# qwertyhgb/Prostate-Cancer-Multimodal-Segmentation

Measured on AMD Instinct MI355X. Metric: train volumes/sec (5ch 128x128x64), higher is better.
Workload: dtype bf16; 1 GPU; UNet3D 5->1, 2 x 5x128x128x64 per GPU, BCEDiceLoss, Adam(1e-4, wd 1e-5); global_batch=2, parallelism=dp1

## Files before the change

include/pcms_hip.h:

```cpp
#ifndef PCMS_HIP_H
#define PCMS_HIP_H
#include <hip/hip_runtime.h>

#ifdef __cplusplus
extern "C" {
#endif

#define PCMS_CONV_ACCUMULATE 1
#define PCMS_CONV_RELU 2
#define PCMS_GRAD_STORE 1
#define PCMS_STEM_DENSE 16

int pcms_pack_input(int dtype, const float* in, void* out, int N, int Cin, long V, int Cp, hipStream_t s);

int pcms_conv3_chunk(int dtype);
int pcms_conv3_pack_elems(int dtype, int J, int Kdim);
int pcms_conv3_mblocks(int N, int D, int H, int W);
int pcms_conv3_fwd_rows(int dtype, int N, int D, int H, int W, int c0, int c1, int Cout);
int pcms_conv3_big_min_boxes(int v);
int pcms_conv3_big_max_wgs(int v);
int pcms_conv3_small_box_mtw2(int v);
int pcms_conv3_fwd_box_vol(int v);
int pcms_conv3_pack(int dtype, const float* w, void* out, int Cout, int Cin, int flip, hipStream_t s);
int pcms_conv3_pack2(int dtype, const float* w, void* fwd, void* dgrad, int Cout, int Cin, hipStream_t s);
// ... 75 lines not shown
int pcms_maxpool_fwd(int dtype, const void* a, void* p, int N, int D, int H, int W, int C, hipStream_t s);
int pcms_maxpool_bwd(int dtype, const void* a, const void* dp, void* da, int N, int D, int H, int W,
                     int C, hipStream_t s);
int pcms_bn_relu_pool(int dtype, const void* y, void* a, void* p, const float* scale, const float* shift,
                      int N, int D, int H, int W, int C, hipStream_t s);
int pcms_maxpool_bwd_bn_rows(int dtype, int N, int D, int H, int W, int C);
int pcms_maxpool_bwd_bn(int dtype, const void* y, const float* scale, const float* shift, const float* mean,
                        const float* invstd, const void* dp, void* da, float* part, int N, int D, int H, int W,
                        int C, hipStream_t s);
int pcms_maxpool_bwd_bn_sums(int dtype, const void* y, const float* scale, const float* shift, const float* mean,
                             const float* invstd, const void* dp, const void* da, float* part, int N, int D, int H,
                             int W, int C, hipStream_t s);
int pcms_maxpool_bn_apply(int dtype, const void* y, const float* scale, const float* shift, const float* mean,
                          const float* invstd, const float* coef, const void* dp, const void* da, void* dy, int N,
                          int D, int H, int W, int C, hipStream_t s);

int pcms_convt_fwd_stream(int v);
int pcms_convt_pack_elems(int dtype, int Cin, int Cout);
int pcms_convt_pack(int dtype, const float* w, void* out, int Cin, int Cout, int dgrad, hipStream_t s);
int pcms_convt_fwd(int dtype, const void* x, const void* wpack, const float* bias, void* out,
                   int N, int Din, int Hin, int Win, int Cin, int Cout, int Do, int Ho, int Wo, hipStream_t s);
int pcms_convt_fwd_ws_floats(int N, int Din, int Hin, int Win, int Cin, int Cout);
int pcms_convt_fwd_ws(int dtype, const void* x, const void* wpack, const float* bias, void* out, float* ws,
                      int N, int Din, int Hin, int Win, int Cin, int Cout, int Do, int Ho, int Wo, hipStream_t s);
int pcms_convt_dgrad(int dtype, const void* dout, const void* wpack_d, void* dx,
                     int N, int Din, int Hin, int Win, int Cin, int Cout, int Do, int Ho, int Wo, hipStream_t s);
int pcms_convt_dgrad_ws_floats(int N, int Din, int Hin, int Win, int Cin, int Cout);
int pcms_convt_dgrad_ws(int dtype, const void* dout, const void* wpack_d, void* dx, float* ws,
                        int N, int Din, int Hin, int Win, int Cin, int Cout, int Do, int Ho, int Wo, hipStream_t s);
int pcms_convt_wgrad_ws_floats(int N, int Din, int Hin, int Win, int Cin, int Cout, int target_wgs);
// ... 89 lines not shown
```

prostate-cancer-multimodal-segmentation_amd/_lib.py:

```python
from __future__ import annotations

import ctypes
import os

import torch

LIB_PATH = os.environ.get("PCMS_LIB") or os.path.join(os.path.dirname(os.path.abspath(__file__)), "libpcms_hip.so")

F32, BF16, F32X3 = 0, 1, 2

SIGNATURES = {
    "pcms_pack_input": "ippiilis",
    "pcms_conv3_chunk": "i",
    "pcms_conv3_pack_elems": "iii",
    "pcms_conv3_mblocks": "iiii",
    "pcms_conv3_fwd_rows": "iiiiiiii",
    "pcms_conv3_big_min_boxes": "i",
    "pcms_conv3_big_max_wgs": "i",
    "pcms_conv3_fwd_box_vol": "i",
    "pcms_conv3_small_box_mtw2": "i",
    "pcms_conv3_pack": "ippiiis",
    "pcms_conv3_pack2": "ipppiis",
    "pcms_conv3_splits": "iii",
    "pcms_conv3_fwd": "ipipippppippiiiiiiis",
# ... 32 lines not shown
    "pcms_split_epilogue": "ipipppipilis",
    "pcms_bn_ws_doubles": "i",
    "pcms_bn_finalize": "piidpppppffppppps",
    "pcms_bn_eval_coeffs": "ppppfipps",
    "pcms_bn_fold": "ppppppfilpps",
    "pcms_bn_relu": "ippppils",
    "pcms_bn_bwd_rows": "iil",
    "pcms_bn_relu_bwd": "i" + "p" * 12 + "ilps",
    "pcms_maxpool_fwd": "ippiiiiis",
    "pcms_maxpool_bwd": "ipppiiiiis",
    "pcms_bn_relu_pool": "ipppppiiiiis",
    "pcms_maxpool_bwd_bn_rows": "iiiiii",
    "pcms_maxpool_bwd_bn": "ippppppppiiiiis",
    "pcms_maxpool_bwd_bn_sums": "ippppppppiiiiis",
    "pcms_maxpool_bn_apply": "ipppppppppiiiiis",
    "pcms_bn_relu_bwd_finish": "i" + "p" * 8 + "ippppilps",
    "pcms_convt_pack": "ippiiis",
    "pcms_convt_pack_elems": "iii",
    "pcms_convt_fwd_stream": "i",
    "pcms_convt_fwd": "ippppiiiiiiiiis",
    "pcms_convt_fwd_ws_floats": "iiiiii",
    "pcms_convt_fwd_ws": "ipppppiiiiiiiiis",
    "pcms_convt_dgrad": "ipppiiiiiiiiis",
    "pcms_convt_dgrad_ws_floats": "iiiiii",
    "pcms_convt_dgrad_ws": "ippppiiiiiiiiis",
    "pcms_convt_wgrad_ws_floats": "iiiiiii",
    "pcms_convt_wgrad_taps": "i",
    "pcms_convt_reduce_fused": "i",
    "pcms_bn_bwd_rows_cap": "i",
    "pcms_convt_wgrad": "ippppiiiiiiiiiis",
# ... 111 lines not shown
```

prostate-cancer-multimodal-segmentation_amd/csrc/ops.hip:

```cpp
#include "common.h"
#include "pcms_hip.h"
#include <algorithm>

namespace {

constexpr int TPB = 256;

template <typename T>
__global__ void pack_input_kernel(const float* in, T* out, int N, int Cin, long V, int Cp) {
  const long total = (long)N * V;
  for (long i = blockIdx.x * (long)blockDim.x + threadIdx.x; i < total; i += (long)gridDim.x * blockDim.x) {
    const long n = i / V, v = i % V;
    for (int c = 0; c < Cp; ++c) {
      const float x = c < Cin ? in[(n * Cin + c) * V + v] : 0.f;
      Elem<T>::st(out + i * Cp + c, x);
    }
  }
}

template <typename T>
__global__ void __launch_bounds__(256) pack_input4_kernel(const float* in, T* out, int N, int Cin, long V) {
  const long quads = (long)N * V / 4;
  for (long i = blockIdx.x * (long)blockDim.x + threadIdx.x; i < quads; i += (long)gridDim.x * blockDim.x) {
    const long n = (4 * i) / V, v = (4 * i) % V;
// ... 371 lines not shown
      for (int j = 0; j < VEC; ++j)
        if (v[j] > m[j] || (v[j] != v[j] && m[j] == m[j])) { m[j] = v[j]; arg[j] = k; }
    }
    float g[VEC];
    load16<T>(dp + i * VEC, g);
    for (int k = 0; k < 8; ++k) {
      float o[VEC];
      load16<T>(da + vin[k] * C + cv * VEC, o);
#pragma unroll
      for (int j = 0; j < VEC; ++j) o[j] += (arg[j] == k) ? g[j] : 0.f;
      store16<T>(da + vin[k] * C + cv * VEC, o);
    }
  }
}

template <typename T, bool NT>
__global__ void __launch_bounds__(TPB) bn_relu_pool_kernel(const T* y, T* a, T* p, const float* scale,
                                                           const float* shift, int N, int D, int H, int W,
                                                           int C) {
  constexpr int VEC = Elem<T>::kVec;
  const int Dc = (D + 1) / 2, Hc = (H + 1) / 2, Wc = (W + 1) / 2, CV = C / VEC;
  const int Do = D / 2, Ho = H / 2, Wo = W / 2;
  const long total = (long)N * Dc * Hc * Wc * CV;
  const long stride = (long)gridDim.x * blockDim.x;
  long i = blockIdx.x * (long)blockDim.x + threadIdx.x;
  const int cv = (int)(i % CV);
  float sc[VEC], sh[VEC];
#pragma unroll
  for (int j = 0; j < VEC; ++j) { sc[j] = scale[cv * VEC + j]; sh[j] = shift[cv * VEC + j]; }
  for (; i < total; i += stride) {
    uint32_t r = (uint32_t)(i / CV);
    const int wc = r % Wc; r /= Wc;
    const int hc = r % Hc; r /= Hc;
    const int dc = r % Dc; const long n = r / Dc;
    float m[VEC];
#pragma unroll
    for (int j = 0; j < VEC; ++j) m[j] = -INFINITY;
    float v[8][VEC];
    long vin[8];
    bool in[8];
#pragma unroll
    for (int k = 0; k < 8; ++k) {
      const int d = 2 * dc + (k >> 2), h = 2 * hc + ((k >> 1) & 1), w = 2 * wc + (k & 1);
      in[k] = d < D && h < H && w < W;
      vin[k] = ((n * D + d) * H + h) * W + w;
#ifndef BRP_NTLOAD
#define BRP_NTLOAD 1
#endif
      if (in[k]) ld16<NT && BRP_NTLOAD>(y + vin[k] * C + cv * VEC, v[k]);
    }
#pragma unroll
    for (int k = 0; k < 8; ++k) {
      if (!in[k]) continue;
#pragma unroll
      for (int j = 0; j < VEC; ++j) v[k][j] = round_st<T>(bn_relu1(v[k][j], sc[j], sh[j]));
      st16<NT>(a + vin[k] * C + cv * VEC, v[k]);
#pragma unroll
      for (int j = 0; j < VEC; ++j)
        if (v[k][j] > m[j] || v[k][j] != v[k][j]) m[j] = v[k][j];
    }
    if (dc < Do && hc < Ho && wc < Wo) store16<T>(p + (((n * Do + dc) * Ho + hc) * Wo + wc) * C + cv * VEC, m);
  }
}

template <typename T, bool STORE = true>
__global__ void __launch_bounds__(TPB, 3) maxpool_bwd_bn_kernel(const T* y, const float* scale, const float* shift,
                                                             const float* mean, const float* invstd, const T* dp,
                                                             T* da, float* part, int N, int D, int H, int W,
                                                             int C) {
  constexpr int VEC = Elem<T>::kVec;
  __shared__ float red[TPB][VEC][2];
  const int Dc = (D + 1) / 2, Hc = (H + 1) / 2, Wc = (W + 1) / 2, CV = C / VEC;
  const int Do = D / 2, Ho = H / 2, Wo = W / 2;
  const long total = (long)N * Dc * Hc * Wc * CV;
  const long stride = (long)gridDim.x * blockDim.x;
  long i = blockIdx.x * (long)blockDim.x + threadIdx.x;
  const int cv = (int)(i % CV);
  float sc[VEC], sh[VEC], mu[VEC], is[VEC], sg[VEC], sgx[VEC];
#pragma unroll
  for (int j = 0; j < VEC; ++j) {
    const int c = cv * VEC + j;
    sc[j] = scale[c]; sh[j] = shift[c]; mu[j] = mean[c]; is[j] = invstd[c];
    sg[j] = 0.f; sgx[j] = 0.f;
  }
// ... 14 lines not shown
    const bool whole = dc < Do && hc < Ho && wc < Wo;
    u32x4_t yr[8], dr[8], gr = {0u, 0u, 0u, 0u};
    const long v0 = ((n * D + 2 * dc) * H + 2 * hc) * W + 2 * wc;
    const bool ind = 2 * dc + 1 < D, inh = 2 * hc + 1 < H, inw = 2 * wc + 1 < W;
    auto vk = [&](int k) { return v0 + (long)(k >> 2) * H * W + ((k >> 1) & 1) * W + (k & 1); };
    auto ink = [&](int k) { return (!(k & 4) || ind) && (!(k & 2) || inh) && (!(k & 1) || inw); };
#pragma unroll
    for (int k = 0; k < 8; ++k) {
      yr[k] = (u32x4_t){0u, 0u, 0u, 0u};
      dr[k] = yr[k];
      if (ink(k)) {
        yr[k] = *reinterpret_cast<const u32x4_t*>(y + vk(k) * C + cv * VEC);
        dr[k] = *reinterpret_cast<const u32x4_t*>(da + vk(k) * C + cv * VEC);
      }
    }
    if (whole) gr = *reinterpret_cast<const u32x4_t*>(dp + (((n * Do + dc) * Ho + hc) * Wo + wc) * C + cv * VEC);
    float g[VEC], m[VEC];
    int arg[VEC];
    unpack(gr, g);
#pragma unroll
    for (int j = 0; j < VEC; ++j) { m[j] = -INFINITY; arg[j] = 0; }
    auto round2 = [](f32x2_t v) -> f32x2_t {
      if constexpr (sizeof(T) == 2) {
        const uint32_t u = pack_bf16x2(v[0], v[1]);
        return (f32x2_t){__uint_as_float(u << 16), __uint_as_float(u & 0xffff0000u)};
      } else {
        return v;
      }
    };
    auto z2of = [&](const float (&yv)[VEC], int q) {
      return __builtin_elementwise_fma((f32x2_t){yv[2 * q], yv[2 * q + 1]}, (f32x2_t){sc[2 * q], sc[2 * q + 1]},
                                       (f32x2_t){sh[2 * q], sh[2 * q + 1]});
    };
    if (whole) {
#pragma unroll
      for (int k = 0; k < 8; ++k) {
        float yv[VEC];
        unpack(yr[k], yv);
#pragma unroll
        for (int j = 0; j < VEC; ++j) {
          const float av = round_st<T>(bn_relu1(yv[j], sc[j], sh[j]));
          if (av > m[j] || (av != av && m[j] == m[j])) { m[j] = av; arg[j] = k; }
        }
      }
    }
#pragma unroll
    for (int k = 0; k < 8; ++k) {
      if (!ink(k)) continue;
      float yv[VEC], o[VEC];
// ... 111 lines not shown
    for (int k = 0; k < 8; ++k) {
      if (!ink(k)) continue;
      float yv[VEC], o[VEC], out[VEC];
      u32x4_t yk = yr[k];
      asm volatile("" : "+v"(yk));
      unpack(yk, yv);
      unpack(dr[k], o);
      if (whole) {
#pragma unroll
        for (int j = 0; j < VEC; ++j) o[j] = round_st<T>(o[j] + ((arg[j] == k) ? g[j] : 0.f));
      }
#pragma unroll
      for (int j = 0; j < VEC; ++j) out[j] = bn_bwd_dy(o[j], yv[j], sc[j], sh[j], mu[j], is[j], k1[j], k2[j], k3[j]);
      st16<NT>(dy + vk(k) * C + cv * VEC, out);
    }
  }
}

template <typename T>
__global__ void __launch_bounds__(TPB) box_channel_sum_kernel(const T* x, float* part, int N, int D, int H, int W,
                                                              int C, int z0, int y0, int x0, int bd, int bh, int bw) {
  constexpr int VEC = Elem<T>::kVec;
  __shared__ float red[TPB * VEC];
  const int CG = C / VEC;
  const int cg = threadIdx.x % CG, vl = threadIdx.x / CG, VL = TPB / CG;
  const long nv = (long)N * bd * bh * bw;
  float acc[VEC];
#pragma unroll
  for (int j = 0; j < VEC; ++j) acc[j] = 0.f;
  const long stride = (long)gridDim.x * VL;
// ... 833 lines not shown
  if (e != hipSuccess || dy == nullptr) return (int)e;
  const int grid = ew_grid(dtype, C, nvox);
  if (dtype == PCMS_BF16)
    hipLaunchKernelGGL((nt ? bn_relu_bwd_apply_kernel<bf16_t, true> : bn_relu_bwd_apply_kernel<bf16_t, false>), dim3(grid), dim3(TPB), 0, s, (const bf16_t*)da, (const bf16_t*)y, scale, shift, mean, invstd, (const float*)coef, (bf16_t*)dy, C, nvox);
  else
    hipLaunchKernelGGL((nt ? bn_relu_bwd_apply_kernel<float, true> : bn_relu_bwd_apply_kernel<float, false>), dim3(grid), dim3(TPB), 0, s, (const float*)da, (const float*)y, scale, shift, mean, invstd, (const float*)coef, (float*)dy, C, nvox);
  PCMS_CHECK_LAUNCH();
}

static int cell_grid(long total, int CV, int cap) {
  int g = grid_for(total, TPB, cap);
  const int per = CV / std::__gcd(CV, TPB);
  return std::max(per, g / per * per);
}

int pcms_bn_relu_pool(int dtype, const void* y, void* a, void* p, const float* scale, const float* shift, int N,
                      int D, int H, int W, int C, hipStream_t s) {
  const int VEC = dtype == PCMS_BF16 ? 8 : 4;
  if (C % VEC) return -1;
  const long cells = (long)N * ((D + 1) / 2) * ((H + 1) / 2) * ((W + 1) / 2);
  if (cells * 8 >= (1L << 31)) return -7;
  const int CV = C / VEC;
  const int grid = cell_grid(cells * CV, CV, 8192);
  const bool nt = (long)N * D * H * W * C * (dtype == PCMS_BF16 ? 2 : 4) >= kNtBytesBn;
  if (dtype == PCMS_BF16)
    hipLaunchKernelGGL((nt ? bn_relu_pool_kernel<bf16_t, true> : bn_relu_pool_kernel<bf16_t, false>), dim3(grid),
                       dim3(TPB), 0, s, (const bf16_t*)y, (bf16_t*)a, (bf16_t*)p, scale, shift, N, D, H, W, C);
  else
    hipLaunchKernelGGL((nt ? bn_relu_pool_kernel<float, true> : bn_relu_pool_kernel<float, false>), dim3(grid),
                       dim3(TPB), 0, s, (const float*)y, (float*)a, (float*)p, scale, shift, N, D, H, W, C);
  PCMS_CHECK_LAUNCH();
}

int pcms_maxpool_bwd_bn_rows(int dtype, int N, int D, int H, int W, int C) {
  const int VEC = dtype == PCMS_BF16 ? 8 : 4;
  const long cells = (long)N * ((D + 1) / 2) * ((H + 1) / 2) * ((W + 1) / 2);
  return cell_grid(cells * (C / VEC), C / VEC, g_bn_rows_cap);
}

int pcms_maxpool_bwd_bn(int dtype, const void* y, const float* scale, const float* shift, const float* mean,
                        const float* invstd, const void* dp, void* da, float* part, int N, int D, int H, int W,
                        int C, hipStream_t s) {
  const int VEC = dtype == PCMS_BF16 ? 8 : 4;
  if (C % VEC || TPB % (C / VEC)) return -1;
  const long cells = (long)N * ((D + 1) / 2) * ((H + 1) / 2) * ((W + 1) / 2);
  if (cells * 8 >= (1L << 31)) return -7;
  const int grid = pcms_maxpool_bwd_bn_rows(dtype, N, D, H, W, C);
  if (dtype == PCMS_BF16)
    hipLaunchKernelGGL(maxpool_bwd_bn_kernel<bf16_t>, dim3(grid), dim3(TPB), 0, s, (const bf16_t*)y, scale, shift,
                       mean, invstd, (const bf16_t*)dp, (bf16_t*)da, part, N, D, H, W, C);
  else
    hipLaunchKernelGGL(maxpool_bwd_bn_kernel<float>, dim3(grid), dim3(TPB), 0, s, (const float*)y, scale, shift,
                       mean, invstd, (const float*)dp, (float*)da, part, N, D, H, W, C);
  PCMS_CHECK_LAUNCH();
}

int pcms_maxpool_bwd_bn_sums(int dtype, const void* y, const float* scale, const float* shift, const float* mean,
                             const float* invstd, const void* dp, const void* da, float* part, int N, int D, int H,
                             int W, int C, hipStream_t s) {
  const int VEC = dtype == PCMS_BF16 ? 8 : 4;
  if (C % VEC || TPB % (C / VEC)) return -1;
  const long cells = (long)N * ((D + 1) / 2) * ((H + 1) / 2) * ((W + 1) / 2);
  if (cells * 8 >= (1L << 31)) return -7;
  const int grid = pcms_maxpool_bwd_bn_rows(dtype, N, D, H, W, C);
  if (dtype == PCMS_BF16)
    hipLaunchKernelGGL((maxpool_bwd_bn_kernel<bf16_t, false>), dim3(grid), dim3(TPB), 0, s, (const bf16_t*)y, scale,
                       shift, mean, invstd, (const bf16_t*)dp, (bf16_t*)const_cast<void*>(da), part, N, D, H, W, C);
  else
    hipLaunchKernelGGL((maxpool_bwd_bn_kernel<float, false>), dim3(grid), dim3(TPB), 0, s, (const float*)y, scale,
                       shift, mean, invstd, (const float*)dp, (float*)const_cast<void*>(da), part, N, D, H, W, C);
  PCMS_CHECK_LAUNCH();
}

int pcms_maxpool_bn_apply(int dtype, const void* y, const float* scale, const float* shift, const float* mean,
                          const float* invstd, const float* coef, const void* dp, const void* da, void* dy, int N,
                          int D, int H, int W, int C, hipStream_t s) {
  const int VEC = dtype == PCMS_BF16 ? 8 : 4;
  if (C % VEC || TPB % (C / VEC)) return -1;
  const long cells = (long)N * ((D + 1) / 2) * ((H + 1) / 2) * ((W + 1) / 2);
  if (cells * 8 >= (1L << 31)) return -7;
  const int CV = C / VEC;
  const int grid = cell_grid(cells * CV, CV, 8192);
  const bool nt = (long)N * D * H * W * C * (dtype == PCMS_BF16 ? 2 : 4) >= kNtBytesBn;
  if (dtype == PCMS_BF16)
    hipLaunchKernelGGL((nt ? maxpool_bn_apply_kernel<bf16_t, true> : maxpool_bn_apply_kernel<bf16_t, false>),
                       dim3(grid), dim3(TPB), 0, s, (const bf16_t*)y, scale, shift, mean, invstd, coef,
                       (const bf16_t*)dp, (const bf16_t*)da, (bf16_t*)dy, N, D, H, W, C);
  else
    hipLaunchKernelGGL((nt ? maxpool_bn_apply_kernel<float, true> : maxpool_bn_apply_kernel<float, false>),
                       dim3(grid), dim3(TPB), 0, s, (const float*)y, scale, shift, mean, invstd, coef,
                       (const float*)dp, (const float*)da, (float*)dy, N, D, H, W, C);
  PCMS_CHECK_LAUNCH();
}

int pcms_maxpool_fwd(int dtype, const void* a, void* p, int N, int D, int H, int W, int C, hipStream_t s) {
  if ((long)N * D * H * W * C >= (1L << 31)) return -7;
  const int VEC = dtype == PCMS_BF16 ? 8 : 4;
  const long total = (long)N * (D / 2) * (H / 2) * (W / 2) * (C / VEC);
  const int grid = grid_for(total, TPB);
  if (dtype == PCMS_BF16) hipLaunchKernelGGL(maxpool_fwd_kernel<bf16_t>, dim3(grid), dim3(TPB), 0, s, (const bf16_t*)a, (bf16_t*)p, N, D, H, W, C);
  else hipLaunchKernelGGL(maxpool_fwd_kernel<float>, dim3(grid), dim3(TPB), 0, s, (const float*)a, (float*)p, N, D, H, W, C);
  PCMS_CHECK_LAUNCH();
}

int pcms_maxpool_bwd(int dtype, const void* a, const void* dp, void* da, int N, int D, int H, int W, int C,
                     hipStream_t s) {
// ... 231 lines not shown
```

prostate-cancer-multimodal-segmentation_amd/engine.py:

```python
from __future__ import annotations

import contextlib
import math
import os
from typing import Dict, List, NamedTuple, Optional, Tuple

import torch

from . import _lib
from ._lib import BF16, F32, F32X3, call, query
from .dp import module_grad_ranges

BN_EPS = 1e-5
BN_MOMENTUM = 0.1

_DT = {"bf16": (torch.bfloat16, BF16), "fp32": (torch.float32, F32)}


class Route(NamedTuple):
    kind: str
    splits: int
    slabs: int
    slabs16: int
    rows: int
    pack16: bool


class Layout(NamedTuple):
    N: int
    D: int
    H: int
    W: int
    act_ckpt: bool
    side_min_level: int
    convt_wgrad_side: bool
    pool_bn_apply_fused: bool
    wgrad_target: int
    split_target: int
    fuse_bnin: bool
    use_b16: bool
    switches: Tuple[int, ...]
    fwd: Tuple[Route, ...] = ()
    dgrad: Tuple[Optional[Route], ...] = ()
    bnin: Tuple[bool, ...] = ()
    pool_rows: Tuple[int, ...] = ()


class ConvSpec:
    __slots__ = ("mod", "cin", "cout", "cin_store", "fwd", "dgrad", "code", "fwd16", "dgrad16", "old_stale",
                 "old_used", "i")

# ... 84 lines not shown
        self.bufs = None
        self.buf_key = None
        self.layout: Optional[Layout] = None
        self.epoch = 0
        self.saved_epoch = -1
        self.saved_eval_epoch = -1
        self._folded = False
        self.act_ckpt = False
        self.split_target = 512
        self.wgrad_target = 256
        self.grad_ready = None
        self.kernel_timer = None
        self.wgrad_side_min_level = 99
        self.convt_wgrad_side = False
        self.pool_bn_apply_fused = False
        self._side_stream = None
        self._side_used = False
        self.fold_bn_eval = True
        self._eval = None
        self._eval_key = None
        self._bn_epoch = 0
        self._wgen = 0
        self._store_ranges = None
        self._gstore = False
        self._flatten()
        for bn in self.bns:
            c = bn.c
            bn.scale, bn.shift, bn.mean, bn.invstd = (torch.empty(c, device=device) for _ in range(4))

    def set_fp32_conv_mode(self, mode: str, convs=None):
# ... 390 lines not shown
        if min(S[4]) < 1:
            raise ValueError(f"spatial size {(D, H, W)} is too small for 4 poolings")
        nv = [N * d * h * w for (d, h, w) in S]
        C = [64 * (1 << l) for l in range(5)]
        T = self.tdtype
        dev = self.device

        def act(l, c):
            return torch.empty(nv[l] * c, dtype=T, device=dev)

        b: Dict[str, object] = {"S": S, "nv": nv, "C": C}
        b["xin"] = act(0, self.cp)
        for l in range(5):
            if l > 0:
                b[f"pool{l}"] = act(l, C[l - 1])
            for k in ("y1", "a1", "y2", "x"):
                b[f"e{l}_{k}"] = act(l, C[l])
        for l in range(4):
            for k in (("u", "a2") if L.act_ckpt else ("u", "y1", "a1", "y2", "a2")):
                b[f"d{l}_{k}"] = act(l, C[l]) if (l, k) != (0, "a2") else None
        if L.act_ckpt:
            for k in ("y1", "a1", "y2"):
                b[f"ck_{k}"] = act(0, C[0])
        for l in range(5):
            b[f"gx{l}"] = act(l, C[l])
            b[f"gA{l}"] = act(l, C[l])
            b[f"gY{l}"] = act(l, C[l])
            b[f"gZ{l}"] = act(l, C[l]) if l >= L.side_min_level else b[f"gY{l}"]
            b[f"gU{l}"] = act(l, C[l])
        self.stem_sup = query("pcms_stem_supported", N, D, H, W) if self.stem_fast else 0
# ... 106 lines not shown
        if recompute:
            return
        m = bn.mod
        if training:
            if nvox <= 1:
                raise ValueError(f"Expected more than 1 value per channel when training, got input size "
                                 f"torch.Size([{N}, {bn.c}, {S[0]}, {S[1]}, {S[2]}])")
            call("pcms_bn_finalize", st, r.rows, bn.c, float(nvox), m.weight, m.bias, m.running_mean,
                 m.running_var, m.num_batches_tracked, BN_MOMENTUM, BN_EPS, bn.scale, bn.shift, bn.mean,
                 bn.invstd, b["bnws"])
        else:
            call("pcms_bn_eval_coeffs", m.weight, m.bias, m.running_mean, m.running_var, BN_EPS, bn.c,
                 bn.scale, bn.shift)

    def _block_fwd(self, blk: BlockSpec, x0, c0, x1, c1, out: Dict[str, torch.Tensor], N, S, training,
                   recompute: bool = False, pool_out=None):
        nvox = N * S[0] * S[1] * S[2]
        if not training and self._folded:
            i0 = blk.c0.i
            a2 = out["a2"] if out["a2"] is not None else out["y2"]
            self._conv_eval(i0, x0, c0, x1, c1, out["a1"], N, S)
            self._conv_eval(i0 + 1, out["a1"], blk.c0.cout, None, 0, a2, N, S)
            if pool_out is not None:
                call("pcms_maxpool_fwd", self.code, a2, pool_out, N, *S, blk.c1.cout)
            return
        self._conv(blk.c0, x0, c0, x1, c1, out["y1"], N, S, True, training, blk.b0, recompute)
        if self.layout.bnin[blk.c0.i // 2]:
            self._conv(blk.c1, out["y1"], blk.c0.cout, None, 0, out["y2"], N, S, True, training, blk.b1, recompute,
                       bnin=blk.b0)
        else:
            call("pcms_bn_relu", self.code, out["y1"], out["a1"], blk.b0.scale, blk.b0.shift, blk.c0.cout, nvox)
            self._conv(blk.c1, out["a1"], blk.c0.cout, None, 0, out["y2"], N, S, True, training, blk.b1, recompute)
        if recompute or out["a2"] is None:
            return
        if pool_out is not None:
            call("pcms_bn_relu_pool", self.code, out["y2"], out["a2"], pool_out, blk.b1.scale, blk.b1.shift, N, *S,
                 blk.c1.cout)
        else:
            call("pcms_bn_relu", self.code, out["y2"], out["a2"], blk.b1.scale, blk.b1.shift, blk.c1.cout, nvox)

    def _dec_acts(self, l: int) -> Dict[str, torch.Tensor]:
        b = self.bufs
        if not self.layout.act_ckpt:
            return {k: b[f"d{l}_{k}"] for k in ("y1", "a1", "y2", "a2")}
        n = b["nv"][l] * b["C"][l]
        return {"y1": b["ck_y1"][:n], "a1": b["ck_a1"][:n], "y2": b["ck_y2"][:n], "a2": b[f"d{l}_a2"]}

    def forward(self, x: torch.Tensor, training: bool, act: int = 0, threshold: float = 0.5,
                keep_input_grad: bool = False) -> torch.Tensor:
        if keep_input_grad and training:
            raise ValueError("keep_input_grad is the eval route; a training forward keeps its activations anyway")
        if x.dim() != 5 or x.shape[1] != self.nmod:
            raise ValueError(f"expected input (N, {self.nmod}, D, H, W), got {tuple(x.shape)}")
        if x.device != self.device:
            raise ValueError(f"input on {x.device}, model on {self.device}")
        x = x.contiguous()
        if x.dtype != torch.float32:
            x = x.float()
        N, _, D, H, W = x.shape
        key = (N, D, H, W, self.act_ckpt, self.wgrad_side_min_level, self.convt_wgrad_side, self.pool_bn_apply_fused,
               self.wgrad_target, self.split_target, self.fuse_bnin, self.use_b16, _lib.switches())
        if key != self.buf_key:
            self._alloc(key)
        self._ensure_packs()
        folded = self._folded = not training and self.fold_bn_eval and not keep_input_grad
        if folded:
            self._ensure_eval_packs()
        else:
            self._bn_epoch += training
        b = self.bufs
        S, C = b["S"], b["C"]
        call("pcms_pack_input", self.code, x, b["xin"], N, self.nmod, D * H * W, self.cp)
        inp, cin = b["xin"], self.cp
        for l in range(5):
            if l > 0:
                inp, cin = b[f"pool{l}"], C[l - 1]
            out = {"y1": b[f"e{l}_y1"], "a1": b[f"e{l}_a1"], "y2": b[f"e{l}_y2"], "a2": b[f"e{l}_x"]}
            self._block_fwd(self.enc[l], inp, cin, None, 0, out, N, S[l], training,
                            pool_out=b[f"pool{l + 1}"] if l < 4 else None)
        h = b["e4_x"]
        for i in range(4):
            l = 3 - i
            up = self.ups[i]
            fpack, _ = self.convt_packs[i]
            call("pcms_convt_fwd_ws", self.code, h, fpack, up.bias, b[f"d{l}_u"], b["ctws"], N, *S[l + 1],
                 up.in_channels, up.out_channels, *S[l])
            self._block_fwd(self.dec[i], b[f"e{l}_x"], C[l], b[f"d{l}_u"], C[l], self._dec_acts(l), N, S[l],
                            training)
            h = b[f"d{l}_a2"]
        logits = torch.empty((N, self.ncls, D, H, W), dtype=torch.float32, device=self.device)
        oc = self.model.outc
        bn = self.dec[3].b1
        if folded:
            call("pcms_head_fwd", self.code, self._dec_acts(0)["y2"], oc.weight, oc.bias, logits, D * H * W, N,
# ... 10 lines not shown

    def _stem_dgrad(self, dy1, N, S) -> torch.Tensor:
        key = (self._wgen, self.flat_p._version)
        if self.stem_dpack is None:
            self.stem_dpack = torch.empty(query("pcms_stem_dgrad_pack_elems", self.code), dtype=self.tdtype,
                                          device=self.device)
        if key != self._stem_dpack_key:
            call("pcms_stem_dgrad_pack", self.code, self.convs[0].mod.weight, self.stem_dpack, self.nmod)
            self._stem_dpack_key = key
        dx = torch.empty((N, self.nmod, *S), dtype=torch.float32, device=self.device)
        with self._timed("stem_dgrad"):
            call("pcms_stem_dgrad", self.code, dy1, self.stem_dpack, dx, N, *S, self.nmod)
        return dx

    def _block_bwd(self, blk: BlockSpec, ga2, acts, x0, c0, x1, c1, gx_out0, gx_out1, cy0, N, S, lvl,
                   bn1_rows: int = 0, pool_dp=None, want_dx: bool = False):
        b = self.bufs
        wt = self.layout.wgrad_target
        nvox = N * S[0] * S[1] * S[2]
        self._join_side()
        gY, gZ, gA = b[f"gY{lvl}"], b[f"gZ{lvl}"], b[f"gA{lvl}"]
        if ga2 is not None and bn1_rows:
            m = blk.b1.mod
            call("pcms_bn_relu_bwd_finish", self.code, ga2, acts["y2"], blk.b1.scale, blk.b1.shift, blk.b1.mean,
                 blk.b1.invstd, m.weight, b["stats"], bn1_rows, b["coef"], m.weight.grad, m.bias.grad,
                 gY if pool_dp is None else None, blk.b1.c, nvox, b["bnws"])
            if pool_dp is not None:
                call("pcms_maxpool_bn_apply", self.code, acts["y2"], blk.b1.scale, blk.b1.shift, blk.b1.mean,
                     blk.b1.invstd, b["coef"], pool_dp, ga2, gY, N, *S, blk.b1.c)
        elif ga2 is not None:
            self._bn_bwd(blk.b1, ga2, acts["y2"], gY, nvox)
        if ga2 is not None:
            self._grads_done(blk.b1.mod.weight, blk.b1.mod.bias)
        with self._side(lvl):
            if self.layout.bnin[blk.c0.i // 2]:
                call("pcms_conv3_wgrad_bnin", blk.c1.code, acts["y1"], blk.c0.cout, blk.b0.scale, blk.b0.shift, gY,
                     blk.c1.mod.weight.grad, b["dwt"], N, *S, blk.c1.cout, blk.c1.cin, wt, int(self._gstore))
            else:
                call("pcms_conv3_wgrad", blk.c1.code, acts["a1"], blk.c0.cout, None, 0, gY, blk.c1.mod.weight.grad,
                     b["dwt"], N, *S, blk.c1.cout, blk.c1.cin, wt, int(self._gstore))
        self._grads_done(blk.c1.mod.weight, blk.c1.mod.bias)
        self._dgrad(blk.c1, gY, gA, None, blk.c1.cin, N, S)
# ... 66 lines not shown
            gu = b[f"gU{l}"]
            self._block_bwd(blk, g, acts, b[f"e{l}_x"], C[l], b[f"d{l}_u"], C[l], b[f"gx{l}"], gu, C[l], N,
                            S[l], l)
            up = self.ups[i]
            _, dpack = self.convt_packs[i]
            hin = b["e4_x"] if i == 0 else b[f"d{l + 1}_a2"]
            with self._side(l, L.convt_wgrad_side):
                call("pcms_convt_wgrad_bias", self.code, hin, gu, up.weight.grad, up.bias.grad,
                     b["ctws_w"] if L.convt_wgrad_side else b["ctws"], b["redws"], N, *S[l + 1], up.in_channels,
                     up.out_channels, *S[l], 512)
            self._grads_done(up.weight, up.bias)
            gnext = b["gx4"] if i == 0 else b[f"gA{l + 1}"]
            call("pcms_convt_dgrad_ws", self.code, gu, dpack, gnext, b["ctws"], N, *S[l + 1], up.in_channels,
                 up.out_channels, *S[l])
            g = gnext
        rows, pool_dp, dx = 0, None, None
        for l in reversed(range(5)):
            blk = self.enc[l]
            acts = {"y1": b[f"e{l}_y1"], "a1": b[f"e{l}_a1"], "y2": b[f"e{l}_y2"]}
            if l == 0:
                dx = self._block_bwd(blk, b["gx0"], acts, b["xin"], self.cp, None, 0, None, None, 0, N, S[0], 0,
                                     bn1_rows=rows, pool_dp=pool_dp, want_dx=want_dx)
            else:
                gp = b[f"gU{l}"]
                self._block_bwd(blk, b[f"gx{l}"], acts, b[f"pool{l}"], C[l - 1], None, 0, gp, None, C[l - 1], N,
                                S[l], l, bn1_rows=rows, pool_dp=pool_dp)
                bn = self.enc[l - 1].b1
                call("pcms_maxpool_bwd_bn_sums" if L.pool_bn_apply_fused else "pcms_maxpool_bwd_bn", self.code,
                     b[f"e{l - 1}_y2"], bn.scale, bn.shift, bn.mean, bn.invstd, gp, b[f"gx{l - 1}"], b["stats"], N,
                     *S[l - 1], C[l - 1])
                pool_dp = gp if L.pool_bn_apply_fused else None
                rows = L.pool_rows[l - 1]
        self._join_side()
        self.saved_epoch = -1
        return dx

    def _block_bwd_input(self, blk: BlockSpec, ga2, acts, gx_out0, gx_out1, cy0, N, S, lvl, stem: bool = False):
        b = self.bufs
        nvox = N * S[0] * S[1] * S[2]
        gY, gZ, gA = b[f"gY{lvl}"], b[f"gZ{lvl}"], b[f"gA{lvl}"]
        if ga2 is not None:
            call("pcms_bn_relu_bwd_eval", self.code, ga2, acts["y2"], blk.b1.scale, blk.b1.shift, gY, blk.b1.c, nvox)
        self._dgrad(blk.c1, gY, gA, None, blk.c1.cin, N, S)
        call("pcms_bn_relu_bwd_eval", self.code, gA, acts["y1"], blk.b0.scale, blk.b0.shift, gZ, blk.b0.c, nvox)
        if stem:
            return self._stem_dgrad(gZ, N, S)
# ... 44 lines not shown
```

Measured before the change: 161.0 volumes/s.

## Store maxpool argmax indices in forward and reuse them in pooled BN backward

The fused BN+ReLU+maxpool forward now also writes a per-element uint8 argmax index for each 2x2x2 window. The backward pool/BN kernels read that index instead of re-reading all eight y values and recomputing BN+ReLU to find the max location. A new index-aware apply kernel routes the pooled gradient using the stored index. This trades an extra index buffer write and read, plus slightly more forward work, for less backward memory traffic and compute.

```diff
diff --git a/include/pcms_hip.h b/include/pcms_hip.h
--- a/include/pcms_hip.h
+++ b/include/pcms_hip.h
@@ -1,6 +1,7 @@
 #ifndef PCMS_HIP_H
 #define PCMS_HIP_H
 #include <hip/hip_runtime.h>
+#include <stdint.h>
 
 #ifdef __cplusplus
 extern "C" {
@@ -113,6 +114,14 @@
 int pcms_maxpool_bn_apply(int dtype, const void* y, const float* scale, const float* shift, const float* mean,
                           const float* invstd, const float* coef, const void* dp, const void* da, void* dy, int N,
                           int D, int H, int W, int C, hipStream_t s);
+int pcms_bn_relu_pool_idx(int dtype, const void* y, void* a, void* p, uint8_t* idx, const float* scale,
+                          const float* shift, int N, int D, int H, int W, int C, hipStream_t s);
+int pcms_maxpool_bwd_bn_sums_idx(int dtype, const void* y, const float* scale, const float* shift, const float* mean,
+                                 const float* invstd, const void* dp, const uint8_t* idx, const void* da, float* part,
+                                 int N, int D, int H, int W, int C, hipStream_t s);
+int pcms_maxpool_bn_apply_idx(int dtype, const void* y, const float* scale, const float* shift, const float* mean,
+                              const float* invstd, const float* coef, const void* dp, const uint8_t* idx,
+                              const void* da, void* dy, int N, int D, int H, int W, int C, hipStream_t s);
 
 int pcms_convt_fwd_stream(int v);
 int pcms_convt_pack_elems(int dtype, int Cin, int Cout);
diff --git a/prostate-cancer-multimodal-segmentation_amd/_lib.py b/prostate-cancer-multimodal-segmentation_amd/_lib.py
--- a/prostate-cancer-multimodal-segmentation_amd/_lib.py
+++ b/prostate-cancer-multimodal-segmentation_amd/_lib.py
@@ -70,6 +70,9 @@
     "pcms_maxpool_bwd_bn": "ippppppppiiiiis",
     "pcms_maxpool_bwd_bn_sums": "ippppppppiiiiis",
     "pcms_maxpool_bn_apply": "ipppppppppiiiiis",
+    "pcms_bn_relu_pool_idx": "ippppppiiiiis",
+    "pcms_maxpool_bwd_bn_sums_idx": "ipppppppppiiiiis",
+    "pcms_maxpool_bn_apply_idx": "ippppppppppiiiiis",
     "pcms_bn_relu_bwd_finish": "i" + "p" * 8 + "ippppilps",
     "pcms_convt_pack": "ippiiis",
     "pcms_convt_pack_elems": "iii",
diff --git a/prostate-cancer-multimodal-segmentation_amd/csrc/ops.hip b/prostate-cancer-multimodal-segmentation_amd/csrc/ops.hip
--- a/prostate-cancer-multimodal-segmentation_amd/csrc/ops.hip
+++ b/prostate-cancer-multimodal-segmentation_amd/csrc/ops.hip
@@ -409,8 +409,8 @@
   }
 }
 
-template <typename T, bool NT>
-__global__ void __launch_bounds__(TPB) bn_relu_pool_kernel(const T* y, T* a, T* p, const float* scale,
+template <typename T, bool NT, bool IDX = false>
+__global__ void __launch_bounds__(TPB) bn_relu_pool_kernel(const T* y, T* a, T* p, uint8_t* idx, const float* scale,
                                                            const float* shift, int N, int D, int H, int W,
                                                            int C) {
   constexpr int VEC = Elem<T>::kVec;
@@ -429,8 +429,9 @@
     const int hc = r % Hc; r /= Hc;
     const int dc = r % Dc; const long n = r / Dc;
     float m[VEC];
-#pragma unroll
-    for (int j = 0; j < VEC; ++j) m[j] = -INFINITY;
+    uint32_t arg[VEC];
+#pragma unroll
+    for (int j = 0; j < VEC; ++j) { m[j] = -INFINITY; arg[j] = 0u; }
     float v[8][VEC];
     long vin[8];
     bool in[8];
@@ -444,25 +445,102 @@
 #endif
       if (in[k]) ld16<NT && BRP_NTLOAD>(y + vin[k] * C + cv * VEC, v[k]);
     }
-#pragma unroll
-    for (int k = 0; k < 8; ++k) {
-      if (!in[k]) continue;
-#pragma unroll
-      for (int j = 0; j < VEC; ++j) v[k][j] = round_st<T>(bn_relu1(v[k][j], sc[j], sh[j]));
-      st16<NT>(a + vin[k] * C + cv * VEC, v[k]);
-#pragma unroll
-      for (int j = 0; j < VEC; ++j)
-        if (v[k][j] > m[j] || v[k][j] != v[k][j]) m[j] = v[k][j];
-    }
-    if (dc < Do && hc < Ho && wc < Wo) store16<T>(p + (((n * Do + dc) * Ho + hc) * Wo + wc) * C + cv * VEC, m);
-  }
-}
-
-template <typename T, bool STORE = true>
+    const bool whole = dc < Do && hc < Ho && wc < Wo;
+    const long po = (((n * Do + dc) * Ho + hc) * Wo + wc) * C + cv * VEC;
+    if constexpr (IDX && sizeof(T) == 2) {
+      uint32_t key[VEC], orw = 0u;
+#pragma unroll
+      for (int j = 0; j < VEC; ++j) key[j] = 0u;
+#pragma unroll
+      for (int k = 0; k < 8; ++k) {
+        if (!in[k]) continue;
+        u32x4_t w;
+#pragma unroll
+        for (int q = 0; q < 4; ++q) {
+          w[q] = pack_bf16x2(bn_relu1(v[k][2 * q], sc[2 * q], sh[2 * q]),
+                             bn_relu1(v[k][2 * q + 1], sc[2 * q + 1], sh[2 * q + 1]));
+          orw |= w[q];
+          key[2 * q] = max(key[2 * q], (w[q] << 16) | (uint32_t)(7 - k));
+          key[2 * q + 1] = max(key[2 * q + 1], (w[q] & 0xffff0000u) | (uint32_t)(7 - k));
+        }
+        u32x4_t* ap = reinterpret_cast<u32x4_t*>(a + vin[k] * C + cv * VEC);
+        if constexpr (NT) __builtin_nontemporal_store(w, ap);
+        else *ap = w;
+      }
+      if (whole) {
+        bool odd = (orw & 0x80008000u) != 0u;
+#pragma unroll
+        for (int j = 0; j < VEC; ++j) odd |= key[j] > 0x7f800007u;
+        u32x4_t pw;
+        uint32_t iw[2];
+        if (!odd) {
+#pragma unroll
+          for (int q = 0; q < 4; ++q) pw[q] = (key[2 * q] >> 16) | (key[2 * q + 1] & 0xffff0000u);
+#pragma unroll
+          for (int q = 0; q < 2; ++q)
+            iw[q] = 0x07070707u - ((key[4 * q] & 7u) | ((key[4 * q + 1] & 7u) << 8) |
+                                   ((key[4 * q + 2] & 7u) << 16) | ((key[4 * q + 3] & 7u) << 24));
+        } else {
+#pragma unroll
+          for (int j = 0; j < VEC; ++j) { m[j] = -INFINITY; arg[j] = 0u; }
+#pragma unroll
+          for (int k = 0; k < 8; ++k) {
+            float yv[VEC];
+            load16<T>(y + vin[k] * C + cv * VEC, yv);
+#pragma unroll
+            for (int j = 0; j < VEC; ++j) {
+              const float av = round_st<T>(bn_relu1(yv[j], sc[j], sh[j]));
+              if (av > m[j] || (av != av && m[j] == m[j])) arg[j] = (uint32_t)k;
+              if (av > m[j] || av != av) m[j] = av;
+            }
+          }
+#pragma unroll
+          for (int q = 0; q < 4; ++q) pw[q] = (uint32_t)f2bf(m[2 * q]) | ((uint32_t)f2bf(m[2 * q + 1]) << 16);
+#pragma unroll
+          for (int q = 0; q < 2; ++q)
+            iw[q] = arg[4 * q] | (arg[4 * q + 1] << 8) | (arg[4 * q + 2] << 16) | (arg[4 * q + 3] << 24);
+        }
+        *reinterpret_cast<u32x4_t*>(p + po) = pw;
+        *reinterpret_cast<u32x2_t*>(idx + po) = (u32x2_t){iw[0], iw[1]};
+      }
+    } else {
+#pragma unroll
+      for (int k = 0; k < 8; ++k) {
+        if (!in[k]) continue;
+#pragma unroll
+        for (int j = 0; j < VEC; ++j) v[k][j] = round_st<T>(bn_relu1(v[k][j], sc[j], sh[j]));
+        st16<NT>(a + vin[k] * C + cv * VEC, v[k]);
+#pragma unroll
+        for (int j = 0; j < VEC; ++j) {
+          if constexpr (IDX) {
+            const bool upd = (v[k][j] > m[j]) | (v[k][j] != v[k][j]);
+            arg[j] = (upd & (m[j] == m[j])) ? (uint32_t)k : arg[j];
+            m[j] = upd ? v[k][j] : m[j];
+          } else {
+            if (v[k][j] > m[j] || v[k][j] != v[k][j]) m[j] = v[k][j];
+          }
+        }
+      }
+      if (whole) {
+        store16<T>(p + po, m);
+        if constexpr (IDX) {
+          uint32_t w[VEC / 4];
+#pragma unroll
+          for (int q = 0; q < VEC / 4; ++q)
+            w[q] = arg[4 * q] | (arg[4 * q + 1] << 8) | (arg[4 * q + 2] << 16) | (arg[4 * q + 3] << 24);
+          if constexpr (VEC == 8) *reinterpret_cast<u32x2_t*>(idx + po) = (u32x2_t){w[0], w[1]};
+          else *reinterpret_cast<uint32_t*>(idx + po) = w[0];
+        }
+      }
+    }
+  }
+}
+
+template <typename T, bool STORE = true, bool IDX = false>
 __global__ void __launch_bounds__(TPB, 3) maxpool_bwd_bn_kernel(const T* y, const float* scale, const float* shift,
                                                              const float* mean, const float* invstd, const T* dp,
-                                                             T* da, float* part, int N, int D, int H, int W,
-                                                             int C) {
+                                                             const uint8_t* idx, T* da, float* part, int N, int D,
+                                                             int H, int W, int C) {
   constexpr int VEC = Elem<T>::kVec;
   __shared__ float red[TPB][VEC][2];
   const int Dc = (D + 1) / 2, Hc = (H + 1) / 2, Wc = (W + 1) / 2, CV = C / VEC;
@@ -507,12 +585,27 @@
         dr[k] = *reinterpret_cast<const u32x4_t*>(da + vk(k) * C + cv * VEC);
       }
     }
-    if (whole) gr = *reinterpret_cast<const u32x4_t*>(dp + (((n * Do + dc) * Ho + hc) * Wo + wc) * C + cv * VEC);
+    const long po = (((n * Do + dc) * Ho + hc) * Wo + wc) * C + cv * VEC;
+    uint32_t ir[VEC / 4] = {};
+    if (whole) {
+      gr = *reinterpret_cast<const u32x4_t*>(dp + po);
+      if constexpr (IDX) {
+        if constexpr (VEC == 8) {
+          const u32x2_t t = *reinterpret_cast<const u32x2_t*>(idx + po);
+          ir[0] = t[0]; ir[1] = t[1];
+        } else {
+          ir[0] = *reinterpret_cast<const uint32_t*>(idx + po);
+        }
+      }
+    }
     float g[VEC], m[VEC];
     int arg[VEC];
     unpack(gr, g);
 #pragma unroll
-    for (int j = 0; j < VEC; ++j) { m[j] = -INFINITY; arg[j] = 0; }
+    for (int j = 0; j < VEC; ++j) {
+      m[j] = -INFINITY;
+      arg[j] = IDX ? (int)((ir[j / 4] >> (8 * (j % 4))) & 0xffu) : 0;
+    }
     auto round2 = [](f32x2_t v) -> f32x2_t {
       if constexpr (sizeof(T) == 2) {
         const uint32_t u = pack_bf16x2(v[0], v[1]);
@@ -525,7 +618,7 @@
       return __builtin_elementwise_fma((f32x2_t){yv[2 * q], yv[2 * q + 1]}, (f32x2_t){sc[2 * q], sc[2 * q + 1]},
                                        (f32x2_t){sh[2 * q], sh[2 * q + 1]});
     };
-    if (whole) {
+    if (whole && !IDX) {
 #pragma unroll
       for (int k = 0; k < 8; ++k) {
         float yv[VEC];
@@ -667,6 +760,66 @@
       for (int j = 0; j < VEC; ++j) out[j] = bn_bwd_dy(o[j], yv[j], sc[j], sh[j], mu[j], is[j], k1[j], k2[j], k3[j]);
       st16<NT>(dy + vk(k) * C + cv * VEC, out);
     }
+  }
+}
+
+template <typename T, bool NT>
+__global__ void __launch_bounds__(TPB) maxpool_bn_apply_idx_kernel(
+    const T* y, const float* scale, const float* shift, const float* mean, const float* invstd, const float* coef,
+    const T* dp, const uint8_t* idx, const T* gx, T* dy, int N, int D, int H, int W, int C) {
+  constexpr int VEC = Elem<T>::kVec;
+  const int CG = C / VEC;
+  const int cg = threadIdx.x % CG, vl = threadIdx.x / CG, VL = TPB / CG;
+  const int c0 = cg * VEC;
+  const int Do = D / 2, Ho = H / 2, Wo = W / 2;
+  const long nvox = (long)N * D * H * W;
+  float sc[VEC], sh[VEC], mu[VEC], is[VEC], k1[VEC], k2[VEC], k3[VEC];
+#pragma unroll
+  for (int j = 0; j < VEC; ++j) {
+    const int c = c0 + j;
+    sc[j] = scale[c]; sh[j] = shift[c]; mu[j] = mean[c]; is[j] = invstd[c];
+    k1[j] = coef[c * 3]; k2[j] = coef[c * 3 + 1]; k3[j] = coef[c * 3 + 2];
+  }
+  const uint32_t stride = gridDim.x * (uint32_t)VL;
+  uint32_t r = blockIdx.x * (uint32_t)VL + vl;
+  long v = r;
+  int w = r % W; r /= W;
+  int h = r % H; r /= H;
+  int d = r % D; int n = r / D;
+  uint32_t q = stride;
+  const int sw = q % W; q /= W;
+  const int sh_ = q % H; q /= H;
+  const int sd = q % D; const int sn = q / D;
+  for (; v < nvox; v += stride) {
+    float dv[VEC], yv[VEC], o[VEC];
+    ld16<NT>(gx + v * C + c0, dv);
+    ld16<NT>(y + v * C + c0, yv);
+    if ((d >> 1) < Do && (h >> 1) < Ho && (w >> 1) < Wo) {
+      const long po = ((((long)n * Do + (d >> 1)) * Ho + (h >> 1)) * Wo + (w >> 1)) * C + c0;
+      const uint32_t pos = ((d & 1) << 2) | ((h & 1) << 1) | (w & 1);
+      float g[VEC];
+      load16<T>(dp + po, g);
+      uint32_t ir[VEC / 4];
+      if constexpr (VEC == 8) {
+        const u32x2_t t = *reinterpret_cast<const u32x2_t*>(idx + po);
+        ir[0] = t[0]; ir[1] = t[1];
+      } else {
+        ir[0] = *reinterpret_cast<const uint32_t*>(idx + po);
+      }
+#pragma unroll
+      for (int j = 0; j < VEC; ++j)
+        dv[j] = round_st<T>(dv[j] + ((((ir[j / 4] >> (8 * (j % 4))) & 0xffu) == pos) ? g[j] : 0.f));
+    }
+#pragma unroll
+    for (int j = 0; j < VEC; ++j) o[j] = bn_bwd_dy(dv[j], yv[j], sc[j], sh[j], mu[j], is[j], k1[j], k2[j], k3[j]);
+    st16<NT>(dy + v * C + c0, o);
+    w += sw;
+    int cy = w >= W; w -= cy ? W : 0;
+    h += sh_ + cy;
+    cy = h >= H; h -= cy ? H : 0;
+    d += sd + cy;
+    cy = d >= D; d -= cy ? D : 0;
+    n += sn + cy;
   }
 }
 
@@ -1530,8 +1683,8 @@
   return std::max(per, g / per * per);
 }
 
-int pcms_bn_relu_pool(int dtype, const void* y, void* a, void* p, const float* scale, const float* shift, int N,
-                      int D, int H, int W, int C, hipStream_t s) {
+static int bn_relu_pool_launch(int dtype, const void* y, void* a, void* p, uint8_t* idx, const float* scale,
+                               const float* shift, int N, int D, int H, int W, int C, hipStream_t s) {
   const int VEC = dtype == PCMS_BF16 ? 8 : 4;
   if (C % VEC) return -1;
   const long cells = (long)N * ((D + 1) / 2) * ((H + 1) / 2) * ((W + 1) / 2);
@@ -1540,12 +1693,27 @@
   const int grid = cell_grid(cells * CV, CV, 8192);
   const bool nt = (long)N * D * H * W * C * (dtype == PCMS_BF16 ? 2 : 4) >= kNtBytesBn;
   if (dtype == PCMS_BF16)
-    hipLaunchKernelGGL((nt ? bn_relu_pool_kernel<bf16_t, true> : bn_relu_pool_kernel<bf16_t, false>), dim3(grid),
-                       dim3(TPB), 0, s, (const bf16_t*)y, (bf16_t*)a, (bf16_t*)p, scale, shift, N, D, H, W, C);
+    hipLaunchKernelGGL((idx ? (nt ? bn_relu_pool_kernel<bf16_t, true, true> : bn_relu_pool_kernel<bf16_t, false, true>)
+                            : (nt ? bn_relu_pool_kernel<bf16_t, true> : bn_relu_pool_kernel<bf16_t, false>)),
+                       dim3(grid), dim3(TPB), 0, s, (const bf16_t*)y, (bf16_t*)a, (bf16_t*)p, idx, scale, shift, N, D,
+                       H, W, C);
   else
-    hipLaunchKernelGGL((nt ? bn_relu_pool_kernel<float, true> : bn_relu_pool_kernel<float, false>), dim3(grid),
-                       dim3(TPB), 0, s, (const float*)y, (float*)a, (float*)p, scale, shift, N, D, H, W, C);
-  PCMS_CHECK_LAUNCH();
+    hipLaunchKernelGGL((idx ? (nt ? bn_relu_pool_kernel<float, true, true> : bn_relu_pool_kernel<float, false, true>)
+                            : (nt ? bn_relu_pool_kernel<float, true> : bn_relu_pool_kernel<float, false>)),
+                       dim3(grid), dim3(TPB), 0, s, (const float*)y, (float*)a, (float*)p, idx, scale, shift, N, D, H,
+                       W, C);
+  PCMS_CHECK_LAUNCH();
+}
+
+int pcms_bn_relu_pool(int dtype, const void* y, void* a, void* p, const float* scale, const float* shift, int N,
+                      int D, int H, int W, int C, hipStream_t s) {
+  return bn_relu_pool_launch(dtype, y, a, p, nullptr, scale, shift, N, D, H, W, C, s);
+}
+
+int pcms_bn_relu_pool_idx(int dtype, const void* y, void* a, void* p, uint8_t* idx, const float* scale,
+                          const float* shift, int N, int D, int H, int W, int C, hipStream_t s) {
+  if (!idx) return -2;
+  return bn_relu_pool_launch(dtype, y, a, p, idx, scale, shift, N, D, H, W, C, s);
 }
 
 int pcms_maxpool_bwd_bn_rows(int dtype, int N, int D, int H, int W, int C) {
@@ -1564,28 +1732,44 @@
   const int grid = pcms_maxpool_bwd_bn_rows(dtype, N, D, H, W, C);
   if (dtype == PCMS_BF16)
     hipLaunchKernelGGL(maxpool_bwd_bn_kernel<bf16_t>, dim3(grid), dim3(TPB), 0, s, (const bf16_t*)y, scale, shift,
-                       mean, invstd, (const bf16_t*)dp, (bf16_t*)da, part, N, D, H, W, C);
+                       mean, invstd, (const bf16_t*)dp, (const uint8_t*)nullptr, (bf16_t*)da, part, N, D, H, W, C);
   else
     hipLaunchKernelGGL(maxpool_bwd_bn_kernel<float>, dim3(grid), dim3(TPB), 0, s, (const float*)y, scale, shift,
-                       mean, invstd, (const float*)dp, (float*)da, part, N, D, H, W, C);
-  PCMS_CHECK_LAUNCH();
-}
-
-int pcms_maxpool_bwd_bn_sums(int dtype, const void* y, const float* scale, const float* shift, const float* mean,
-                             const float* invstd, const void* dp, const void* da, float* part, int N, int D, int H,
-                             int W, int C, hipStream_t s) {
+                       mean, invstd, (const float*)dp, (const uint8_t*)nullptr, (float*)da, part, N, D, H, W, C);
+  PCMS_CHECK_LAUNCH();
+}
+
+static int maxpool_bwd_bn_sums_launch(int dtype, const void* y, const float* scale, const float* shift,
+                                      const float* mean, const float* invstd, const void* dp, const uint8_t* idx,
+                                      const void* da, float* part, int N, int D, int H, int W, int C, hipStream_t s) {
   const int VEC = dtype == PCMS_BF16 ? 8 : 4;
   if (C % VEC || TPB % (C / VEC)) return -1;
   const long cells = (long)N * ((D + 1) / 2) * ((H + 1) / 2) * ((W + 1) / 2);
   if (cells * 8 >= (1L << 31)) return -7;
   const int grid = pcms_maxpool_bwd_bn_rows(dtype, N, D, H, W, C);
   if (dtype == PCMS_BF16)
-    hipLaunchKernelGGL((maxpool_bwd_bn_kernel<bf16_t, false>), dim3(grid), dim3(TPB), 0, s, (const bf16_t*)y, scale,
-                       shift, mean, invstd, (const bf16_t*)dp, (bf16_t*)const_cast<void*>(da), part, N, D, H, W, C);
+    hipLaunchKernelGGL((idx ? maxpool_bwd_bn_kernel<bf16_t, false, true> : maxpool_bwd_bn_kernel<bf16_t, false>),
+                       dim3(grid), dim3(TPB), 0, s, (const bf16_t*)y, scale, shift, mean, invstd, (const bf16_t*)dp, idx,
+                       (bf16_t*)const_cast<void*>(da), part, N, D, H, W, C);
   else
-    hipLaunchKernelGGL((maxpool_bwd_bn_kernel<float, false>), dim3(grid), dim3(TPB), 0, s, (const float*)y, scale,
-                       shift, mean, invstd, (const float*)dp, (float*)const_cast<void*>(da), part, N, D, H, W, C);
-  PCMS_CHECK_LAUNCH();
+    hipLaunchKernelGGL((idx ? maxpool_bwd_bn_kernel<float, false, true> : maxpool_bwd_bn_kernel<float, false>),
+                       dim3(grid), dim3(TPB), 0, s, (const float*)y, scale, shift, mean, invstd, (const float*)dp, idx,
+                       (float*)const_cast<void*>(da), part, N, D, H, W, C);
+  PCMS_CHECK_LAUNCH();
+}
+
+int pcms_maxpool_bwd_bn_sums(int dtype, const void* y, const float* scale, const float* shift, const float* mean,
+                             const float* invstd, const void* dp, const void* da, float* part, int N, int D, int H,
+                             int W, int C, hipStream_t s) {
+  return maxpool_bwd_bn_sums_launch(dtype, y, scale, shift, mean, invstd, dp, nullptr, da, part, N, D, H, W, C,
+                                           s);
+}
+
+int pcms_maxpool_bwd_bn_sums_idx(int dtype, const void* y, const float* scale, const float* shift, const float* mean,
+                                 const float* invstd, const void* dp, const uint8_t* idx, const void* da, float* part,
+                                 int N, int D, int H, int W, int C, hipStream_t s) {
+  if (!idx) return -2;
+  return maxpool_bwd_bn_sums_launch(dtype, y, scale, shift, mean, invstd, dp, idx, da, part, N, D, H, W, C, s);
 }
 
 int pcms_maxpool_bn_apply(int dtype, const void* y, const float* scale, const float* shift, const float* mean,
@@ -1606,6 +1790,27 @@
     hipLaunchKernelGGL((nt ? maxpool_bn_apply_kernel<float, true> : maxpool_bn_apply_kernel<float, false>),
                        dim3(grid), dim3(TPB), 0, s, (const float*)y, scale, shift, mean, invstd, coef,
                        (const float*)dp, (const float*)da, (float*)dy, N, D, H, W, C);
+  PCMS_CHECK_LAUNCH();
+}
+
+int pcms_maxpool_bn_apply_idx(int dtype, const void* y, const float* scale, const float* shift, const float* mean,
+                              const float* invstd, const float* coef, const void* dp, const uint8_t* idx,
+                              const void* da, void* dy, int N, int D, int H, int W, int C, hipStream_t s) {
+  const int VEC = dtype == PCMS_BF16 ? 8 : 4;
+  if ((dtype != PCMS_BF16 && dtype != PCMS_F32) || C <= 0 || C % VEC || TPB % (C / VEC)) return -1;
+  if (!y || !dp || !idx || !da || !dy) return -2;
+  const long nvox = (long)N * D * H * W;
+  if (nvox < 1 || nvox >= (1L << 31)) return -7;
+  const int grid = ew_grid(dtype, C, nvox);
+  const bool nt = nvox * C * (dtype == PCMS_BF16 ? 2 : 4) >= kNtBytesBn;
+  if (dtype == PCMS_BF16)
+    hipLaunchKernelGGL((nt ? maxpool_bn_apply_idx_kernel<bf16_t, true> : maxpool_bn_apply_idx_kernel<bf16_t, false>),
+                       dim3(grid), dim3(TPB), 0, s, (const bf16_t*)y, scale, shift, mean, invstd, coef,
+                       (const bf16_t*)dp, idx, (const bf16_t*)da, (bf16_t*)dy, N, D, H, W, C);
+  else
+    hipLaunchKernelGGL((nt ? maxpool_bn_apply_idx_kernel<float, true> : maxpool_bn_apply_idx_kernel<float, false>),
+                       dim3(grid), dim3(TPB), 0, s, (const float*)y, scale, shift, mean, invstd, coef,
+                       (const float*)dp, idx, (const float*)da, (float*)dy, N, D, H, W, C);
   PCMS_CHECK_LAUNCH();
 }
 
diff --git a/prostate-cancer-multimodal-segmentation_amd/engine.py b/prostate-cancer-multimodal-segmentation_amd/engine.py
--- a/prostate-cancer-multimodal-segmentation_amd/engine.py
+++ b/prostate-cancer-multimodal-segmentation_amd/engine.py
@@ -35,6 +35,7 @@
     side_min_level: int
     convt_wgrad_side: bool
     pool_bn_apply_fused: bool
+    pool_index: bool
     wgrad_target: int
     split_target: int
     fuse_bnin: bool
@@ -149,6 +150,7 @@
         self.wgrad_side_min_level = 99
         self.convt_wgrad_side = False
         self.pool_bn_apply_fused = False
+        self.pool_index = True
         self._side_stream = None
         self._side_used = False
         self.fold_bn_eval = True
@@ -569,6 +571,8 @@
         for l in range(5):
             if l > 0:
                 b[f"pool{l}"] = act(l, C[l - 1])
+                if L.pool_index:
+                    b[f"pidx{l}"] = torch.empty(nv[l] * C[l - 1], dtype=torch.uint8, device=dev)
             for k in ("y1", "a1", "y2", "x"):
                 b[f"e{l}_{k}"] = act(l, C[l])
         for l in range(4):
@@ -705,7 +709,7 @@
                  bn.scale, bn.shift)
 
     def _block_fwd(self, blk: BlockSpec, x0, c0, x1, c1, out: Dict[str, torch.Tensor], N, S, training,
-                   recompute: bool = False, pool_out=None):
+                   recompute: bool = False, pool_out=None, pool_idx=None):
         nvox = N * S[0] * S[1] * S[2]
         if not training and self._folded:
             i0 = blk.c0.i
@@ -724,7 +728,10 @@
             self._conv(blk.c1, out["a1"], blk.c0.cout, None, 0, out["y2"], N, S, True, training, blk.b1, recompute)
         if recompute or out["a2"] is None:
             return
-        if pool_out is not None:
+        if pool_idx is not None:
+            call("pcms_bn_relu_pool_idx", self.code, out["y2"], out["a2"], pool_out, pool_idx, blk.b1.scale,
+                 blk.b1.shift, N, *S, blk.c1.cout)
+        elif pool_out is not None:
             call("pcms_bn_relu_pool", self.code, out["y2"], out["a2"], pool_out, blk.b1.scale, blk.b1.shift, N, *S,
                  blk.c1.cout)
         else:
@@ -750,7 +757,7 @@
             x = x.float()
         N, _, D, H, W = x.shape
         key = (N, D, H, W, self.act_ckpt, self.wgrad_side_min_level, self.convt_wgrad_side, self.pool_bn_apply_fused,
-               self.wgrad_target, self.split_target, self.fuse_bnin, self.use_b16, _lib.switches())
+               self.pool_index, self.wgrad_target, self.split_target, self.fuse_bnin, self.use_b16, _lib.switches())
         if key != self.buf_key:
             self._alloc(key)
         self._ensure_packs()
@@ -768,7 +775,8 @@
                 inp, cin = b[f"pool{l}"], C[l - 1]
             out = {"y1": b[f"e{l}_y1"], "a1": b[f"e{l}_a1"], "y2": b[f"e{l}_y2"], "a2": b[f"e{l}_x"]}
             self._block_fwd(self.enc[l], inp, cin, None, 0, out, N, S[l], training,
-                            pool_out=b[f"pool{l + 1}"] if l < 4 else None)
+                            pool_out=b[f"pool{l + 1}"] if l < 4 else None,
+                            pool_idx=b[f"pidx{l + 1}"] if l < 4 and training and self.layout.pool_index else None)
         h = b["e4_x"]
         for i in range(4):
             l = 3 - i
@@ -809,7 +817,7 @@
         return dx
 
     def _block_bwd(self, blk: BlockSpec, ga2, acts, x0, c0, x1, c1, gx_out0, gx_out1, cy0, N, S, lvl,
-                   bn1_rows: int = 0, pool_dp=None, want_dx: bool = False):
+                   bn1_rows: int = 0, pool_dp=None, pool_idx=None, want_dx: bool = False):
         b = self.bufs
         wt = self.layout.wgrad_target
         nvox = N * S[0] * S[1] * S[2]
@@ -820,7 +828,10 @@
             call("pcms_bn_relu_bwd_finish", self.code, ga2, acts["y2"], blk.b1.scale, blk.b1.shift, blk.b1.mean,
                  blk.b1.invstd, m.weight, b["stats"], bn1_rows, b["coef"], m.weight.grad, m.bias.grad,
                  gY if pool_dp is None else None, blk.b1.c, nvox, b["bnws"])
-            if pool_dp is not None:
+            if pool_idx is not None:
+                call("pcms_maxpool_bn_apply_idx", self.code, acts["y2"], blk.b1.scale, blk.b1.shift, blk.b1.mean,
+                     blk.b1.invstd, b["coef"], pool_dp, pool_idx, ga2, gY, N, *S, blk.b1.c)
+            elif pool_dp is not None:
                 call("pcms_maxpool_bn_apply", self.code, acts["y2"], blk.b1.scale, blk.b1.shift, blk.b1.mean,
                      blk.b1.invstd, b["coef"], pool_dp, ga2, gY, N, *S, blk.b1.c)
         elif ga2 is not None:
@@ -917,22 +928,27 @@
             call("pcms_convt_dgrad_ws", self.code, gu, dpack, gnext, b["ctws"], N, *S[l + 1], up.in_channels,
                  up.out_channels, *S[l])
             g = gnext
-        rows, pool_dp, dx = 0, None, None
+        rows, pool_dp, pool_idx, dx = 0, None, None, None
         for l in reversed(range(5)):
             blk = self.enc[l]
             acts = {"y1": b[f"e{l}_y1"], "a1": b[f"e{l}_a1"], "y2": b[f"e{l}_y2"]}
             if l == 0:
                 dx = self._block_bwd(blk, b["gx0"], acts, b["xin"], self.cp, None, 0, None, None, 0, N, S[0], 0,
-                                     bn1_rows=rows, pool_dp=pool_dp, want_dx=want_dx)
+                                     bn1_rows=rows, pool_dp=pool_dp, pool_idx=pool_idx, want_dx=want_dx)
             else:
                 gp = b[f"gU{l}"]
                 self._block_bwd(blk, b[f"gx{l}"], acts, b[f"pool{l}"], C[l - 1], None, 0, gp, None, C[l - 1], N,
-                                S[l], l, bn1_rows=rows, pool_dp=pool_dp)
+                                S[l], l, bn1_rows=rows, pool_dp=pool_dp, pool_idx=pool_idx)
                 bn = self.enc[l - 1].b1
-                call("pcms_maxpool_bwd_bn_sums" if L.pool_bn_apply_fused else "pcms_maxpool_bwd_bn", self.code,
-                     b[f"e{l - 1}_y2"], bn.scale, bn.shift, bn.mean, bn.invstd, gp, b[f"gx{l - 1}"], b["stats"], N,
-                     *S[l - 1], C[l - 1])
-                pool_dp = gp if L.pool_bn_apply_fused else None
+                if L.pool_index:
+                    pool_idx = b[f"pidx{l}"]
+                    call("pcms_maxpool_bwd_bn_sums_idx", self.code, b[f"e{l - 1}_y2"], bn.scale, bn.shift, bn.mean,
+                         bn.invstd, gp, pool_idx, b[f"gx{l - 1}"], b["stats"], N, *S[l - 1], C[l - 1])
+                else:
+                    call("pcms_maxpool_bwd_bn_sums" if L.pool_bn_apply_fused else "pcms_maxpool_bwd_bn", self.code,
+                         b[f"e{l - 1}_y2"], bn.scale, bn.shift, bn.mean, bn.invstd, gp, b[f"gx{l - 1}"], b["stats"],
+                         N, *S[l - 1], C[l - 1])
+                pool_dp = gp if L.pool_index or L.pool_bn_apply_fused else None
                 rows = L.pool_rows[l - 1]
         self._join_side()
         self.saved_epoch = -1
```

Result: no change. 161.0 volumes/s (-0.0%).
